# AIBluefisher/DReg-NeRF

Hardware: AMD Instinct MI355X
Metric: nerf_pairs_per_sec_regtr_fwd_bwd_128 (higher is better)
Workload: dtype bf16; 1 GPU; RegTR fwd+bwd+AdamW, shell-R synthetic pairs, 128^3 grids, 4 pairs (8 grids) per GPU per step, random-init weights; global_batch_pairs=4, resolution=128, fpn_head=active-set (identical results; rows around occupied voxels), parallelism=dp1

## Files before the change

dreg_nerf_amd/csrc/attention.hip:

```cpp
#include "common.h"

template <typename T> struct Frag;
template <> struct Frag<bf16_t> { bf16x8_t v; };
template <> struct Frag<float> { float v[8]; };

__device__ __forceinline__ f32x4_t mma(const Frag<bf16_t>& a, const Frag<bf16_t>& b, f32x4_t c) {
    return __builtin_amdgcn_mfma_f32_16x16x32_bf16(a.v, b.v, c, 0, 0, 0);
}
__device__ __forceinline__ f32x4_t mma(const Frag<float>& a, const Frag<float>& b, f32x4_t c) {
#pragma unroll
    for (int e = 0; e < 8; ++e) c = __builtin_amdgcn_mfma_f32_16x16x4f32(a.v[e], b.v[e], c, 0, 0, 0);
    return c;
}
__device__ __forceinline__ Frag<bf16_t> frag_row(const char* base, int rs, int row, int k0, bf16_t) {
    Frag<bf16_t> f; f.v = *reinterpret_cast<const bf16x8_t*>(base + row * rs + k0 * 2); return f;
}
__device__ __forceinline__ Frag<float> frag_row(const char* base, int rs, int row, int k0, float) {
    Frag<float> f;
    float4 lo = *reinterpret_cast<const float4*>(base + row * rs + k0 * 4);
    float4 hi = *reinterpret_cast<const float4*>(base + row * rs + k0 * 4 + 16);
    f.v[0] = lo.x; f.v[1] = lo.y; f.v[2] = lo.z; f.v[3] = lo.w; f.v[4] = hi.x; f.v[5] = hi.y; f.v[6] = hi.z; f.v[7] = hi.w;
    return f;
}
__device__ __forceinline__ Frag<bf16_t> frag_glob(const bf16_t* p, bool valid) {
    Frag<bf16_t> f;
    if (valid) f.v = *reinterpret_cast<const bf16x8_t*>(p); else f.v = (bf16x8_t){0, 0, 0, 0, 0, 0, 0, 0};
    return f;
}
__device__ __forceinline__ Frag<float> frag_glob(const float* p, bool valid) {
    Frag<float> f;
#pragma unroll
    for (int e = 0; e < 8; ++e) f.v[e] = valid ? p[e] : 0.f;
    return f;
}
struct AttnArgs {
    const void *q, *k, *v;
    void* o;
    float* lse;
    int Nq, Nk;
    int ldq, ldk, ldv, ldo;
    long hq, hk, hv, ho;
    float scale;
    const void* dout;
    float* dvec;
    void *dq, *dk, *dv;
    const int4* probs;
    int Rq;
};

struct Prob { int Nq, Nk; long q0, k0; };
__device__ __forceinline__ Prob get_prob(const AttnArgs& a) {
    Prob p; p.Nq = a.Nq; p.Nk = a.Nk; p.q0 = 0; p.k0 = 0;
    if (a.probs) { const int4 t = a.probs[blockIdx.z]; p.q0 = t.x; p.Nq = t.y; p.k0 = t.z; p.Nk = t.w; }
    return p;
}

template <typename T> __host__ __device__ constexpr int row_pad() { return sizeof(T) == 2 ? 32 : 16; }
template <typename T, int D>
struct TileRegs {
    static constexpr int GPR = D * sizeof(T) / 16, NL = (64 * GPR + 255) / 256;
    uint4 v[NL];
    __device__ __forceinline__ void fetch(const T* src, long ld, int row0, int nrows_valid, int tid) {
#pragma unroll
        for (int i = 0; i < NL; ++i) {
            const int q = tid + i * 256, r = q / GPR, g = q % GPR;
            v[i] = make_uint4(0, 0, 0, 0);
            if (q < 64 * GPR && row0 + r < nrows_valid) v[i] = *reinterpret_cast<const uint4*>(reinterpret_cast<const char*>(src + (long)(row0 + r) * ld) + g * 16);
        }
    }
    __device__ __forceinline__ void store(char* dst, int rs, int tid) const {
#pragma unroll
        for (int i = 0; i < NL; ++i) {
            const int q = tid + i * 256, r = q / GPR, g = q % GPR;
            if (q < 64 * GPR) *reinterpret_cast<uint4*>(dst + r * rs + g * 16) = v[i];
        }
    }
};
__device__ __forceinline__ Frag<bf16_t> frag_regs(const float (&v)[8], bf16_t) {
    typedef __attribute__((ext_vector_type(4))) uint32_t u32x4_t;
    const u32x4_t w = {f2bf2(v[0], v[1]), f2bf2(v[2], v[3]), f2bf2(v[4], v[5]), f2bf2(v[6], v[7])};
    Frag<bf16_t> f; f.v = __builtin_bit_cast(bf16x8_t, w); return f;
}
__device__ __forceinline__ Frag<float> frag_regs(const float (&v)[8], float) {
    Frag<float> f;
#pragma unroll
    for (int e = 0; e < 8; ++e) f.v[e] = v[e];
    return f;
}
__device__ __forceinline__ Frag<bf16_t> frag_colp(const char* base, int rs, int row_lo, int row_hi, int cb, int lane, bf16_t) {
    typedef __attribute__((address_space(3))) bf16x4_t* lds4_t;
    const int fi = lane & 15;
    const int off = (fi >> 2) * rs + (cb + (fi & 3) * 4) * 2;
    bf16x4_t lo = __builtin_amdgcn_ds_read_tr16_b64_v4i16((lds4_t)(base + row_lo * rs + off));
    bf16x4_t hi = __builtin_amdgcn_ds_read_tr16_b64_v4i16((lds4_t)(base + row_hi * rs + off));
    Frag<bf16_t> f; f.v = (bf16x8_t){lo[0], lo[1], lo[2], lo[3], hi[0], hi[1], hi[2], hi[3]};
    return f;
}
__device__ __forceinline__ Frag<float> frag_colp(const char* base, int rs, int row_lo, int row_hi, int cb, int lane, float) {
    const int fi = lane & 15;
    Frag<float> f;
#pragma unroll
    for (int e = 0; e < 8; ++e) f.v[e] = *reinterpret_cast<const float*>(base + (e < 4 ? row_lo + e : row_hi + e - 4) * rs + (cb + fi) * 4);
    return f;
}
__device__ __forceinline__ void store4(bf16_t* p, float a, float b, float c, float d) { *reinterpret_cast<uint2*>(p) = make_uint2(f2bf2(a, b), f2bf2(c, d)); }
__device__ __forceinline__ void store4(float* p, float a, float b, float c, float d) { *reinterpret_cast<float4*>(p) = make_float4(a, b, c, d); }
__device__ __forceinline__ float group4x_sum(float v) { v += __shfl_xor(v, 16, 64); v += __shfl_xor(v, 32, 64); return v; }
__device__ __forceinline__ float group4x_max(float v) { v = fmaxf(v, __shfl_xor(v, 16, 64)); return fmaxf(v, __shfl_xor(v, 32, 64)); }
constexpr float LOG2E = 1.4426950408889634f, LN2 = 0.6931471805599453f;

template <typename T, int D, bool XYZ>
__global__ __launch_bounds__(256) void attn_fwd_kernel(AttnArgs a)
{
    constexpr int DV = 32;
    constexpr int KRS = D * sizeof(T) + row_pad<T>(), VRS = XYZ ? 16 : DV * sizeof(T) + row_pad<T>();
    extern __shared__ __attribute__((aligned(16))) char smem[];
    constexpr int BUF = 64 * KRS + 64 * VRS;
    const int tid = threadIdx.x, lane = tid & 63, wave = tid >> 6;
    const int h = blockIdx.y;
    const Prob pb = get_prob(a);
    if (blockIdx.x * 64 >= pb.Nq) return;
    const int q0 = blockIdx.x * 64 + wave * 16;
    const T* Q = (const T*)a.q + h * a.hq + pb.q0 * a.ldq;
    const T* K = (const T*)a.k + h * a.hk + pb.k0 * a.ldk;
    const int fr = lane & 15, kg = lane >> 4;

    Frag<T> qf[D / 32];
#pragma unroll
    for (int kk = 0; kk < D / 32; ++kk) qf[kk] = frag_glob(Q + (long)(q0 + fr) * a.ldq + kk * 32 + kg * 8, q0 + fr < pb.Nq);
    const float c2 = a.scale * LOG2E;
    float m = -INFINITY, l = 0.f;
    f32x4_t o[2];
    float o3[3] = {0.f, 0.f, 0.f};
    o[0] = o[1] = (f32x4_t){0.f, 0.f, 0.f, 0.f};

    TileRegs<T, D> rk;
    TileRegs<T, DV> rv;
    float4 rx = make_float4(0, 0, 0, 0);
    const T* Vp = XYZ ? nullptr : (const T*)a.v + h * a.hv + pb.k0 * a.ldv;
    auto fetch = [&](int k0) {
        rk.fetch(K, a.ldk, k0, pb.Nk, tid);
        if constexpr (XYZ) {
            const float* x = (const float*)a.v + pb.k0 * 3;
            rx = make_float4(0, 0, 0, 0);
            if (tid < 64 && k0 + tid < pb.Nk) rx = make_float4(x[(long)(k0 + tid) * 3], x[(long)(k0 + tid) * 3 + 1], x[(long)(k0 + tid) * 3 + 2], 0.f);
        } else {
            rv.fetch(Vp, a.ldv, k0, pb.Nk, tid);
        }
    };
    auto stage = [&](int buf) {
        char* dK = smem + buf * BUF;
        rk.store(dK, KRS, tid);
        if constexpr (XYZ) { if (tid < 64) *reinterpret_cast<float4*>(dK + 64 * KRS + tid * 16) = rx; }
        else rv.store(dK + 64 * KRS, VRS, tid);
    };
    fetch(0);
    stage(0);
    if (64 < pb.Nk) fetch(64);
    for (int k0 = 0, buf = 0; k0 < pb.Nk; k0 += 64, buf ^= 1) {
        __syncthreads();
        if (k0 + 64 < pb.Nk) { stage(buf ^ 1); if (k0 + 128 < pb.Nk) fetch(k0 + 128); }
        const char* sK = smem + buf * BUF;
        const char* sV = sK + 64 * KRS;
        f32x4_t s[4];
#pragma unroll
        for (int t = 0; t < 4; ++t) {
            s[t] = (f32x4_t){0.f, 0.f, 0.f, 0.f};
#pragma unroll
            for (int kk = 0; kk < D / 32; ++kk) s[t] = mma(frag_row(sK, KRS, t * 16 + fr, kk * 32 + kg * 8, T()), qf[kk], s[t]);
        }
        if (k0 + 64 > pb.Nk) {
#pragma unroll
            for (int t = 0; t < 4; ++t)
#pragma unroll
                for (int r = 0; r < 4; ++r)
                    if (k0 + t * 16 + kg * 4 + r >= pb.Nk) s[t][r] = -INFINITY;
        }
        float mx = -INFINITY;
#pragma unroll
        for (int t = 0; t < 4; ++t)
#pragma unroll
            for (int r = 0; r < 4; ++r) mx = fmaxf(mx, s[t][r]);
        mx = group4x_max(mx) * c2;
        const float mn = fmaxf(m, mx);
        const float alpha = __builtin_amdgcn_exp2f(m - mn);
        float sum = 0.f;
#pragma unroll
        for (int t = 0; t < 4; ++t)
#pragma unroll
            for (int r = 0; r < 4; ++r) { s[t][r] = __builtin_amdgcn_exp2f(__builtin_fmaf(s[t][r], c2, -mn)); sum += s[t][r]; }
        l = l * alpha + sum;
        m = mn;
        if constexpr (XYZ) {
#pragma unroll
            for (int c = 0; c < 3; ++c) o3[c] *= alpha;
#pragma unroll
            for (int t = 0; t < 4; ++t)
#pragma unroll
                for (int r = 0; r < 4; ++r) {
                    const float4 x = *reinterpret_cast<const float4*>(sV + (t * 16 + kg * 4 + r) * 16);
                    o3[0] += s[t][r] * x.x; o3[1] += s[t][r] * x.y; o3[2] += s[t][r] * x.z;
                }
        } else {
#pragma unroll
            for (int r = 0; r < 4; ++r) { o[0][r] *= alpha; o[1][r] *= alpha; }
#pragma unroll
            for (int ks = 0; ks < 2; ++ks) {
                const float pv[8] = {s[2 * ks][0], s[2 * ks][1], s[2 * ks][2], s[2 * ks][3], s[2 * ks + 1][0], s[2 * ks + 1][1], s[2 * ks + 1][2], s[2 * ks + 1][3]};
                const Frag<T> pf = frag_regs(pv, T());
#pragma unroll
                for (int u = 0; u < 2; ++u) o[u] = mma(frag_colp(sV, VRS, ks * 32 + kg * 4, ks * 32 + 16 + kg * 4, u * 16, lane, T()), pf, o[u]);
            }
        }
    }
    l = group4x_sum(l);
    const float inv = 1.f / l;
    const int qr = q0 + fr;
    if constexpr (XYZ) {
        const float x = group4x_sum(o3[0]), y = group4x_sum(o3[1]), z = group4x_sum(o3[2]);
        if (kg == 0 && qr < pb.Nq) {
            float* op = (float*)a.o + ((long)h * a.Rq + pb.q0 + qr) * 3;
            op[0] = x * inv; op[1] = y * inv; op[2] = z * inv;
        }
    } else if (qr < pb.Nq) {
        T* op = (T*)a.o + h * a.ho + (pb.q0 + qr) * a.ldo + kg * 4;
#pragma unroll
        for (int u = 0; u < 2; ++u) store4(op + u * 16, o[u][0] * inv, o[u][1] * inv, o[u][2] * inv, o[u][3] * inv);
    }
    if (kg == 0 && qr < pb.Nq) a.lse[(long)h * a.Rq + pb.q0 + qr] = (m + __log2f(l)) * LN2;
}

template <typename T, int D, bool XYZ>
__global__ __launch_bounds__(256, (D > 32 ? 2 : 1)) void attn_bwd_dq_kernel(AttnArgs a)
{
    constexpr int DV = 32;
    constexpr int KRS = D * sizeof(T) + row_pad<T>(), VRS = XYZ ? 16 : DV * sizeof(T) + row_pad<T>();
    extern __shared__ __attribute__((aligned(16))) char smem[];
    constexpr int BUF = 64 * KRS + 64 * VRS;
    const int tid = threadIdx.x, lane = tid & 63, wave = tid >> 6;
    const int h = blockIdx.y;
    const Prob pb = get_prob(a);
    if (blockIdx.x * 64 >= pb.Nq) return;
    const int q0 = blockIdx.x * 64 + wave * 16;
    const T* Q = (const T*)a.q + h * a.hq + pb.q0 * a.ldq;
    const T* K = (const T*)a.k + h * a.hk + pb.k0 * a.ldk;
    const int fr = lane & 15, kg = lane >> 4;
    const int qr = q0 + fr;
    const bool qv = qr < pb.Nq;

    Frag<T> qf[D / 32];
#pragma unroll
    for (int kk = 0; kk < D / 32; ++kk) qf[kk] = frag_glob(Q + (long)qr * a.ldq + kk * 32 + kg * 8, qv);
    const float lse2 = qv ? a.lse[(long)h * a.Rq + pb.q0 + qr] * LOG2E : 0.f;
    float dvec, do3[3] = {0.f, 0.f, 0.f};
    Frag<T> dof;
    if constexpr (!XYZ) {
        const T* dO = (const T*)a.dout + h * a.ho + pb.q0 * a.ldo;
        const T* O = (const T*)a.o + h * a.ho + pb.q0 * a.ldo;
        dof = frag_glob(dO + (long)qr * a.ldo + kg * 8, qv);
        const Frag<T> of = frag_glob(O + (long)qr * a.ldo + kg * 8, qv);
        float part = 0.f;
        if constexpr (sizeof(T) == 2) {
#pragma unroll
            for (int e = 0; e < 8; ++e) part += bf2f((bf16_t)dof.v[e]) * bf2f((bf16_t)of.v[e]);
        } else {
#pragma unroll
            for (int e = 0; e < 8; ++e) part += dof.v[e] * of.v[e];
        }
        dvec = group4x_sum(part);
    } else {
        const float* dO = (const float*)a.dout + ((long)h * a.Rq + pb.q0 + qr) * 3;
        const float* O = (const float*)a.o + ((long)h * a.Rq + pb.q0 + qr) * 3;
        dvec = 0.f;
#pragma unroll
        for (int c = 0; c < 3; ++c) { do3[c] = qv ? dO[c] : 0.f; dvec += do3[c] * (qv ? O[c] : 0.f); }
    }
    if (kg == 0 && qv) a.dvec[(long)h * a.Rq + pb.q0 + qr] = dvec;
    const float c2 = a.scale * LOG2E;
    f32x4_t dq[D / 16];
#pragma unroll
    for (int u = 0; u < D / 16; ++u) dq[u] = (f32x4_t){0.f, 0.f, 0.f, 0.f};

    TileRegs<T, D> rk;
    TileRegs<T, DV> rv;
    float4 rx = make_float4(0, 0, 0, 0);
    const T* Vp = XYZ ? nullptr : (const T*)a.v + h * a.hv + pb.k0 * a.ldv;
    auto fetch = [&](int k0) {
        rk.fetch(K, a.ldk, k0, pb.Nk, tid);
        if constexpr (XYZ) {
            const float* x = (const float*)a.v + pb.k0 * 3;
            rx = make_float4(0, 0, 0, 0);
            if (tid < 64 && k0 + tid < pb.Nk) rx = make_float4(x[(long)(k0 + tid) * 3], x[(long)(k0 + tid) * 3 + 1], x[(long)(k0 + tid) * 3 + 2], 0.f);
        } else {
            rv.fetch(Vp, a.ldv, k0, pb.Nk, tid);
        }
    };
    auto stage = [&](int buf) {
        char* dK = smem + buf * BUF;
        rk.store(dK, KRS, tid);
        if constexpr (XYZ) { if (tid < 64) *reinterpret_cast<float4*>(dK + 64 * KRS + tid * 16) = rx; }
        else rv.store(dK + 64 * KRS, VRS, tid);
    };
    fetch(0);
    stage(0);
    if (64 < pb.Nk) fetch(64);
    for (int k0 = 0, buf = 0; k0 < pb.Nk; k0 += 64, buf ^= 1) {
        __syncthreads();
        if (k0 + 64 < pb.Nk) { stage(buf ^ 1); if (k0 + 128 < pb.Nk) fetch(k0 + 128); }
        const char* sK = smem + buf * BUF;
        const char* sV = sK + 64 * KRS;
#pragma unroll
        for (int ks = 0; ks < 2; ++ks) {
            float dsv[8];
#pragma unroll
            for (int tt = 0; tt < 2; ++tt) {
                const int t = 2 * ks + tt;
                f32x4_t s = (f32x4_t){0.f, 0.f, 0.f, 0.f};
#pragma unroll
                for (int kk = 0; kk < D / 32; ++kk) s = mma(frag_row(sK, KRS, t * 16 + fr, kk * 32 + kg * 8, T()), qf[kk], s);
                f32x4_t dp = (f32x4_t){0.f, 0.f, 0.f, 0.f};
                if constexpr (!XYZ) dp = mma(frag_row(sV, VRS, t * 16 + fr, kg * 8, T()), dof, dp);
                if (k0 + 64 > pb.Nk) {
#pragma unroll
                    for (int r = 0; r < 4; ++r)
                        if (k0 + t * 16 + kg * 4 + r >= pb.Nk) s[r] = -INFINITY;
                }
#pragma unroll
                for (int r = 0; r < 4; ++r) {
                    const int kr = t * 16 + kg * 4 + r;
                    const float p = __builtin_amdgcn_exp2f(__builtin_fmaf(s[r], c2, -lse2));
                    float dpv = dp[r];
                    if constexpr (XYZ) {
                        const float4 x = *reinterpret_cast<const float4*>(sV + kr * 16);
                        dpv = do3[0] * x.x + do3[1] * x.y + do3[2] * x.z;
                    }
                    dsv[tt * 4 + r] = p * (dpv - dvec);
                }
            }
            const Frag<T> df = frag_regs(dsv, T());
#pragma unroll
            for (int u = 0; u < D / 16; ++u) {
                dq[u] = mma(frag_colp(sK, KRS, ks * 32 + kg * 4, ks * 32 + 16 + kg * 4, u * 16, lane, T()), df, dq[u]);
                if (D > 32 && (u & 3) == 3) __builtin_amdgcn_sched_barrier(0);
            }
        }
    }
    if (qv) {
        T* dQ = (T*)a.dq + h * a.hq + (pb.q0 + qr) * a.ldq + kg * 4;
#pragma unroll
        for (int u = 0; u < D / 16; ++u) store4(dQ + u * 16, dq[u][0] * a.scale, dq[u][1] * a.scale, dq[u][2] * a.scale, dq[u][3] * a.scale);
    }
}

template <typename T, int D, bool XYZ>
__global__ __launch_bounds__(256, (D > 32 ? 2 : 1)) void attn_bwd_dkv_kernel(AttnArgs a)
{
    constexpr int DV = 32;
    constexpr int QRS = D * sizeof(T) + row_pad<T>(), ORS = XYZ ? 16 : DV * sizeof(T) + row_pad<T>();
    extern __shared__ __attribute__((aligned(16))) char smem[];
    constexpr int BUF = 64 * QRS + 64 * ORS + 128 * (int)sizeof(float);
    const int tid = threadIdx.x, lane = tid & 63, wave = tid >> 6;
    const int h = blockIdx.y;
    const Prob pb = get_prob(a);
    if (blockIdx.x * 64 >= pb.Nk) return;
    const int key0 = blockIdx.x * 64 + wave * 16;
    const T* Q = (const T*)a.q + h * a.hq + pb.q0 * a.ldq;
    const T* K = (const T*)a.k + h * a.hk + pb.k0 * a.ldk;
    const int fr = lane & 15, kg = lane >> 4;
    const int kr = key0 + fr;
    const bool kv = kr < pb.Nk;

    Frag<T> kf[D / 32], vf;
#pragma unroll
    for (int kk = 0; kk < D / 32; ++kk) kf[kk] = frag_glob(K + (long)kr * a.ldk + kk * 32 + kg * 8, kv);
    float x3[3] = {0.f, 0.f, 0.f};
    if constexpr (!XYZ) {
        vf = frag_glob((const T*)a.v + h * a.hv + (pb.k0 + (long)kr) * a.ldv + kg * 8, kv);
    } else {
#pragma unroll
        for (int c = 0; c < 3; ++c) x3[c] = kv ? ((const float*)a.v)[(pb.k0 + kr) * 3 + c] : 0.f;
    }
    const float c2 = a.scale * LOG2E;
    f32x4_t dk[D / 16], dvv[2];
#pragma unroll
    for (int u = 0; u < D / 16; ++u) dk[u] = (f32x4_t){0.f, 0.f, 0.f, 0.f};
    dvv[0] = dvv[1] = (f32x4_t){0.f, 0.f, 0.f, 0.f};

    TileRegs<T, D> rq;
    TileRegs<T, DV> ro;
    float4 rg = make_float4(0, 0, 0, 0);
    float rl = 0.f, rd = 0.f;
    const T* dOp = XYZ ? nullptr : (const T*)a.dout + h * a.ho + pb.q0 * a.ldo;
    auto fetch = [&](int q0) {
        rq.fetch(Q, a.ldq, q0, pb.Nq, tid);
        if constexpr (XYZ) {
            rg = make_float4(0, 0, 0, 0);
            if (tid < 64 && q0 + tid < pb.Nq) {
                const float* g = (const float*)a.dout + ((long)h * a.Rq + pb.q0 + q0 + tid) * 3;
                rg = make_float4(g[0], g[1], g[2], 0.f);
            }
        } else {
            ro.fetch(dOp, a.ldo, q0, pb.Nq, tid);
        }
        rl = rd = 0.f;
        if (tid < 64 && q0 + tid < pb.Nq) { rl = a.lse[(long)h * a.Rq + pb.q0 + q0 + tid] * LOG2E; rd = a.dvec[(long)h * a.Rq + pb.q0 + q0 + tid]; }
    };
    auto stage = [&](int buf) {
        char* dQ = smem + buf * BUF;
        rq.store(dQ, QRS, tid);
        if constexpr (XYZ) { if (tid < 64) *reinterpret_cast<float4*>(dQ + 64 * QRS + tid * 16) = rg; }
        else ro.store(dQ + 64 * QRS, ORS, tid);
        float* dL = reinterpret_cast<float*>(dQ + 64 * QRS + 64 * ORS);
        if (tid < 64) { dL[tid] = rl; dL[64 + tid] = rd; }
    };
    fetch(0);
    stage(0);
    if (64 < pb.Nq) fetch(64);
    for (int q0 = 0, buf = 0; q0 < pb.Nq; q0 += 64, buf ^= 1) {
        __syncthreads();
        if (q0 + 64 < pb.Nq) { stage(buf ^ 1); if (q0 + 128 < pb.Nq) fetch(q0 + 128); }
        const char* sQ = smem + buf * BUF;
        const char* sO = sQ + 64 * QRS;
        const float* sL = reinterpret_cast<const float*>(sO + 64 * ORS);
#pragma unroll
        for (int ks = 0; ks < 2; ++ks) {
            float pv[8], dsv[8];
#pragma unroll
            for (int tt = 0; tt < 2; ++tt) {
                const int t = 2 * ks + tt;
                f32x4_t s = (f32x4_t){0.f, 0.f, 0.f, 0.f};
#pragma unroll
                for (int kk = 0; kk < D / 32; ++kk) s = mma(frag_row(sQ, QRS, t * 16 + fr, kk * 32 + kg * 8, T()), kf[kk], s);
                f32x4_t dp = (f32x4_t){0.f, 0.f, 0.f, 0.f};
                if constexpr (!XYZ) dp = mma(frag_row(sO, ORS, t * 16 + fr, kg * 8, T()), vf, dp);
                const float4 l4 = *reinterpret_cast<const float4*>(sL + t * 16 + kg * 4);
                const float4 d4 = *reinterpret_cast<const float4*>(sL + 64 + t * 16 + kg * 4);
                const float lq[4] = {l4.x, l4.y, l4.z, l4.w}, dq_[4] = {d4.x, d4.y, d4.z, d4.w};
#pragma unroll
                for (int r = 0; r < 4; ++r) {
                    const int ql = t * 16 + kg * 4 + r;
                    const float p = __builtin_amdgcn_exp2f(__builtin_fmaf(s[r], c2, -lq[r]));
                    float dpv = dp[r];
                    if constexpr (XYZ) {
                        const float4 g = *reinterpret_cast<const float4*>(sO + ql * 16);
                        dpv = x3[0] * g.x + x3[1] * g.y + x3[2] * g.z;
                    }
                    pv[tt * 4 + r] = p;
                    dsv[tt * 4 + r] = p * (dpv - dq_[r]);
                }
            }
            const Frag<T> sf = frag_regs(dsv, T());
#pragma unroll
            for (int u = 0; u < D / 16; ++u) {
                dk[u] = mma(frag_colp(sQ, QRS, ks * 32 + kg * 4, ks * 32 + 16 + kg * 4, u * 16, lane, T()), sf, dk[u]);
                if (D > 32 && (u & 3) == 3) __builtin_amdgcn_sched_barrier(0);
            }
            if constexpr (!XYZ) {
                const Frag<T> pf = frag_regs(pv, T());
#pragma unroll
                for (int u = 0; u < 2; ++u) dvv[u] = mma(frag_colp(sO, ORS, ks * 32 + kg * 4, ks * 32 + 16 + kg * 4, u * 16, lane, T()), pf, dvv[u]);
            }
        }
    }
    if (kv) {
        T* dK = (T*)a.dk + h * a.hk + (pb.k0 + (long)kr) * a.ldk + kg * 4;
#pragma unroll
        for (int u = 0; u < D / 16; ++u) store4(dK + u * 16, dk[u][0] * a.scale, dk[u][1] * a.scale, dk[u][2] * a.scale, dk[u][3] * a.scale);
        if constexpr (!XYZ) {
            T* dV = (T*)a.dv + h * a.hv + (pb.k0 + (long)kr) * a.ldv + kg * 4;
            store4(dV, dvv[0][0], dvv[0][1], dvv[0][2], dvv[0][3]);
            store4(dV + 16, dvv[1][0], dvv[1][1], dvv[1][2], dvv[1][3]);
        }
    }
}

template <typename T, int D, bool XYZ>
static int launch_attn(const AttnArgs& a, int H, int mode, hipStream_t st, int nprob = 1, int maxq = 0, int maxk = 0)
{
    const int gq = ((a.probs ? maxq : a.Nq) + 63) / 64, gk = ((a.probs ? maxk : a.Nk) + 63) / 64;
    constexpr int DV = 32;
    const size_t krs = D * sizeof(T) + row_pad<T>(), vrs = XYZ ? 16 : DV * sizeof(T) + row_pad<T>();
    if (mode == 0) {
        const size_t lds = 2 * (64 * krs + 64 * vrs);
        if (lds > 65536) (void)hipFuncSetAttribute((const void*)attn_fwd_kernel<T, D, XYZ>, hipFuncAttributeMaxDynamicSharedMemorySize, (int)lds);
        hipLaunchKernelGGL((attn_fwd_kernel<T, D, XYZ>), dim3(gq, H, nprob), dim3(256), lds, st, a);
    } else if (mode == 1) {
        const size_t lds = 2 * (64 * krs + 64 * vrs);
        if (lds > 65536) (void)hipFuncSetAttribute((const void*)attn_bwd_dq_kernel<T, D, XYZ>, hipFuncAttributeMaxDynamicSharedMemorySize, (int)lds);
        hipLaunchKernelGGL((attn_bwd_dq_kernel<T, D, XYZ>), dim3(gq, H, nprob), dim3(256), lds, st, a);
    } else {
        const size_t lds = 2 * (64 * krs + 64 * vrs + 128 * sizeof(float));
        if (lds > 65536) (void)hipFuncSetAttribute((const void*)attn_bwd_dkv_kernel<T, D, XYZ>, hipFuncAttributeMaxDynamicSharedMemorySize, (int)lds);
        hipLaunchKernelGGL((attn_bwd_dkv_kernel<T, D, XYZ>), dim3(gk, H, nprob), dim3(256), lds, st, a);
    }
    DREG_LAUNCH_CHECK();
    return DREG_OK;
}

static int dispatch_attn(const AttnArgs& a, int H, int D, int xyz, int dtype, int mode, hipStream_t st, int nprob = 1, int maxq = 0, int maxk = 0)
{
    if (!a.probs && (a.Nq <= 0 || a.Nk <= 0)) return DREG_EINVAL;
    if (a.probs && (nprob <= 0 || maxq <= 0 || maxk <= 0)) return DREG_EINVAL;
    if (D == 32 && !xyz) return dtype == 0 ? launch_attn<bf16_t, 32, false>(a, H, mode, st, nprob, maxq, maxk) : launch_attn<float, 32, false>(a, H, mode, st, nprob, maxq, maxk);
    if (D == 256 && xyz) return dtype == 0 ? launch_attn<bf16_t, 256, true>(a, H, mode, st, nprob, maxq, maxk) : launch_attn<float, 256, true>(a, H, mode, st, nprob, maxq, maxk);
    return DREG_EINVAL;
}

extern "C" {

int dreg_mha_fwd(const void* q, const void* k, const void* v, void* o, float* lse, int Nq, int Nk, int H,
                 int ldq, int ldk, int ldv, int ldo, float scale, int dtype, void* stream)
{
    AttnArgs a = {};
    a.q = q; a.k = k; a.v = v; a.o = o; a.lse = lse; a.Nq = Nq; a.Nk = Nk;
    a.ldq = ldq; a.ldk = ldk; a.ldv = ldv; a.ldo = ldo; a.hq = a.hk = a.hv = a.ho = 32; a.scale = scale; a.Rq = Nq;
    return dispatch_attn(a, H, 32, 0, dtype, 0, (hipStream_t)stream);
}
int dreg_mha_bwd(const void* q, const void* k, const void* v, const void* o, const void* dout, const float* lse,
                 float* dvec, void* dq, void* dk, void* dv, int Nq, int Nk, int H,
                 int ldq, int ldk, int ldv, int ldo, float scale, int dtype, void* stream)
{
    AttnArgs a = {};
    a.q = q; a.k = k; a.v = v; a.o = (void*)o; a.lse = (float*)lse; a.Nq = Nq; a.Nk = Nk;
    a.ldq = ldq; a.ldk = ldk; a.ldv = ldv; a.ldo = ldo; a.hq = a.hk = a.hv = a.ho = 32; a.scale = scale;
    a.dout = dout; a.dvec = dvec; a.dq = dq; a.dk = dk; a.dv = dv; a.Rq = Nq;
    int rc = dispatch_attn(a, H, 32, 0, dtype, 1, (hipStream_t)stream);
    if (rc) return rc;
    return dispatch_attn(a, H, 32, 0, dtype, 2, (hipStream_t)stream);
}
int dreg_corr_attention_fwd(const void* q, const void* k, const float* xyz, float* out, float* lse, int L, int Nq, int Nk,
                            float scale, int dtype, void* stream)
{
    AttnArgs a = {};
    a.q = q; a.k = k; a.v = xyz; a.o = out; a.lse = lse; a.Nq = Nq; a.Nk = Nk;
    a.ldq = a.ldk = 256; a.hq = (long)Nq * 256; a.hk = (long)Nk * 256; a.scale = scale; a.Rq = Nq;
    return dispatch_attn(a, L, 256, 1, dtype, 0, (hipStream_t)stream);
}
int dreg_corr_attention_bwd(const void* q, const void* k, const float* xyz, const float* out, const float* dout,
                            const float* lse, float* dvec, void* dq, void* dk, int L, int Nq, int Nk,
                            float scale, int dtype, void* stream)
{
    AttnArgs a = {};
    a.q = q; a.k = k; a.v = xyz; a.o = (void*)out; a.lse = (float*)lse; a.Nq = Nq; a.Nk = Nk;
    a.ldq = a.ldk = 256; a.hq = (long)Nq * 256; a.hk = (long)Nk * 256; a.scale = scale;
    a.dout = dout; a.dvec = dvec; a.dq = dq; a.dk = dk; a.Rq = Nq;
    int rc = dispatch_attn(a, L, 256, 1, dtype, 1, (hipStream_t)stream);
    if (rc) return rc;
    return dispatch_attn(a, L, 256, 1, dtype, 2, (hipStream_t)stream);
}

int dreg_mha_varlen_fwd(const void* q, const void* k, const void* v, void* o, float* lse, const int* probs, int nprob,
                        int max_q, int max_k, int R, int H, int ldq, int ldk, int ldv, int ldo, float scale, int dtype, void* stream)
{
    AttnArgs a = {};
    a.q = q; a.k = k; a.v = v; a.o = o; a.lse = lse; a.probs = (const int4*)probs; a.Rq = R;
    a.ldq = ldq; a.ldk = ldk; a.ldv = ldv; a.ldo = ldo; a.hq = a.hk = a.hv = a.ho = 32; a.scale = scale;
    return dispatch_attn(a, H, 32, 0, dtype, 0, (hipStream_t)stream, nprob, max_q, max_k);
}
int dreg_mha_varlen_bwd(const void* q, const void* k, const void* v, const void* o, const void* dout, const float* lse,
                        float* dvec, void* dq, void* dk, void* dv, const int* probs, int nprob, int max_q, int max_k, int R, int H,
                        int ldq, int ldk, int ldv, int ldo, float scale, int dtype, void* stream)
{
    AttnArgs a = {};
    a.q = q; a.k = k; a.v = v; a.o = (void*)o; a.lse = (float*)lse; a.probs = (const int4*)probs; a.Rq = R;
    a.ldq = ldq; a.ldk = ldk; a.ldv = ldv; a.ldo = ldo; a.hq = a.hk = a.hv = a.ho = 32; a.scale = scale;
    a.dout = dout; a.dvec = dvec; a.dq = dq; a.dk = dk; a.dv = dv;
    int rc = dispatch_attn(a, H, 32, 0, dtype, 1, (hipStream_t)stream, nprob, max_q, max_k);
    if (rc) return rc;
    return dispatch_attn(a, H, 32, 0, dtype, 2, (hipStream_t)stream, nprob, max_q, max_k);
}
int dreg_corr_attention_varlen_fwd(const void* q, const void* k, const float* xyz, float* out, float* lse, const int* probs, int nprob,
                                   int max_q, int max_k, int L, int R, float scale, int dtype, void* stream)
{
    AttnArgs a = {};
    a.q = q; a.k = k; a.v = xyz; a.o = out; a.lse = lse; a.probs = (const int4*)probs; a.Rq = R;
    a.ldq = a.ldk = 256; a.hq = a.hk = (long)R * 256; a.scale = scale;
    return dispatch_attn(a, L, 256, 1, dtype, 0, (hipStream_t)stream, nprob, max_q, max_k);
}
int dreg_corr_attention_varlen_bwd(const void* q, const void* k, const float* xyz, const float* out, const float* dout,
                                   const float* lse, float* dvec, void* dq, void* dk, const int* probs, int nprob,
                                   int max_q, int max_k, int L, int R, float scale, int dtype, void* stream)
{
    AttnArgs a = {};
    a.q = q; a.k = k; a.v = xyz; a.o = (void*)out; a.lse = (float*)lse; a.probs = (const int4*)probs; a.Rq = R;
    a.ldq = a.ldk = 256; a.hq = a.hk = (long)R * 256; a.scale = scale;
    a.dout = dout; a.dvec = dvec; a.dq = dq; a.dk = dk;
    int rc = dispatch_attn(a, L, 256, 1, dtype, 1, (hipStream_t)stream, nprob, max_q, max_k);
    if (rc) return rc;
    return dispatch_attn(a, L, 256, 1, dtype, 2, (hipStream_t)stream, nprob, max_q, max_k);
}

}
```

dreg_nerf_amd/lib.py:

```python
import ctypes
import os
from ctypes import c_float, c_int, c_size_t, c_void_p

import torch

_HERE = os.path.dirname(os.path.abspath(__file__))
LIB_PATH = os.path.join(_HERE, "libdreg_nerf_hip.so")

DT_BF16 = 0
DT_F32 = 1

_lib = None


class DregError(RuntimeError):
    pass


def _sig(lib, name, restype, argtypes):
    fn = getattr(lib, name)
    fn.restype = restype
    fn.argtypes = argtypes
    return fn

# ... 119 lines not shown
    "dreg_exec_set_timing": (None, [P, I]),
    "dreg_exec_read_timings": (I, [P, P, P, I]),
    "dreg_exec_forward": (I, [P, P, Z, P, P, P, I, I, P]),
    "dreg_exec_backward": (I, [P, P, Z, P, P, P, P, I, P, P]),
    "dreg_exec_backward_range": (I, [P, P, Z, P, P, P, P, I, P, P, I, I, I]),
    "dreg_mha_fwd": (I, [P] * 5 + [I] * 7 + [F, I, P]),
    "dreg_mha_bwd": (I, [P] * 10 + [I] * 7 + [F, I, P]),
    "dreg_corr_attention_fwd": (I, [P] * 5 + [I] * 3 + [F, I, P]),
    "dreg_corr_attention_bwd": (I, [P] * 9 + [I] * 3 + [F, I, P]),
    "dreg_mha_varlen_fwd": (I, [P] * 6 + [I] * 9 + [F, I, P]),
    "dreg_mha_varlen_bwd": (I, [P] * 11 + [I] * 9 + [F, I, P]),
    "dreg_corr_attention_varlen_fwd": (I, [P] * 6 + [I] * 5 + [F, I, P]),
    "dreg_corr_attention_varlen_bwd": (I, [P] * 10 + [I] * 5 + [F, I, P]),
    "dreg_layernorm_fwd": (I, [P] * 6 + [I, I, F, I, P]),
    "dreg_layernorm_bwd_workspace_bytes": (Z, [I]),
    "dreg_layernorm_bwd": (I, [P] * 8 + [I] * 5 + [P]),
    "dreg_layernorm_bwd_add": (I, [P] * 9 + [I] * 4 + [P]),
    "dreg_layernorm_fwd2": (I, [P, P, P, P, I, P, P, P, I, I, F, P]),
    "dreg_layernorm_bwd_parts": (I, [P] * 10 + [I, I, I, P]),
    "dreg_layernorm_bwd_blocks": (I, [I]),
    "dreg_layernorm_bwd_final_batched": (I, [P, I, P]),
    "dreg_overlap_bwd_acc": (I, [P, P, P, P, P, P, P, P, I, P, I, P]),
    "dreg_colsum_rows_per_chunk": (I, [Z]),
    "dreg_colsum_batched": (I, [P, I, I, I, P]),
    "dreg_brick_supported": (I, [I] * 6),
    "dreg_conv3_brick_pack_bytes": (Z, [I, I]),
    "dreg_pack_conv_weight_brick": (I, [P, P, I, I, I, P]),
    "dreg_brick_tiles_workspace_bytes": (Z, [I] * 4),
    "dreg_brick_tiles_build": (I, [P, I, I, I, I, I, I, P, Z, P, P, P, P, P, P]),
    "dreg_conv3_brick": (I, [P, P, P, P, P, P, I, P, P, P] + [I] * 11 + [P]),
    "dreg_ps_num_params": (I, []),
    "dreg_ps_num_linears": (I, []),
    "dreg_ps_create": (P, [P]),
    "dreg_ps_destroy": (None, [P]),
    "dreg_ps_set_fuse": (None, [P, I]),
    "dreg_ps_set_timing": (None, [P, I]),
    "dreg_ps_read_timings": (I, [P, P, P, I]),
    "dreg_ps_arena_bytes": (Z, [P, I]),
    "dreg_ps_panel_fwd": (I, [P] * 13 + [I, I, I, I, F, P]),
    "dreg_ps_panel_bwd": (I, [P] * 12 + [I, I, I, P]),
    "dreg_ps_forward": (I, [P, P, Z, P, P, P, P, P, P, I, I, I, P, P, P, P]),
    "dreg_ps_backward": (I, [P, P, Z, P, P, P, P, P, P, I, I, I, P, P, P, P, P, P, P, P, P, I]),
    "dreg_posenc_sine": (I, [P, P, I, F, F, P]),
    "dreg_overlap_fwd": (I, [P, P, P, P, I, P]),
    "dreg_overlap_bwd_workspace_bytes": (Z, [I]),
    "dreg_overlap_bwd": (I, [P] * 8 + [I, P]),
    "dreg_relu_bwd": (I, [P, P, P, Z, I, I, I, P]),
    "dreg_weighted_kabsch": (I, [P, P, P, P, I, I, F, P]),
    "dreg_weighted_kabsch_pairs": (I, [P, P, P, P, P, I, I, I, F, P]),
    "dreg_weighted_kabsch_bwd": (I, [P] * 7 + [I, I, F, P]),
    "dreg_weighted_kabsch_pairs_bwd": (I, [P] * 7 + [I, I, I, F, P]),
    "dreg_reg_point_losses": (I, [P] * 10 + [I, I, I, I, F, F, F, P]),
    "dreg_infonce_nn": (I, [P] * 7 + [I, I, F, P]),
    "dreg_infonce_rows": (I, [P] * 10 + [I, I, F, F, I, P]),
    "dreg_reg_losses_final": (I, [P] * 6 + [I, I, F, F, F, F, F, P]),
    "dreg_nerf_cont_deferred": (I, [P] * 5 + [I, I, I, F, F, F, F, P]),
    "dreg_halfspace_labels": (I, [P, P, P, P, I, I, P]),
    "dreg_voxel_downsample_workspace_bytes": (Z, [I]),
    "dreg_voxel_downsample_fwd": (I, [P] * 11 + [Z, I, I, I, F, P]),
    "dreg_voxel_downsample_bwd": (I, [P, P, P, P, I, I, P]),
    "dreg_voxel_downsample_plan": (I, [P] * 11 + [Z, I, I, F, P]),
    "dreg_voxel_downsample_plan_frozen": (I, [P] * 11 + [Z, I, I, F, P, P]),
    "dreg_voxel_segment_mean": (I, [P] * 5 + [I, I, P]),
    "dreg_grad_norm": (I, [P, P, P, Z, P]),
    "dreg_adamw_step": (I, [P] * 5 + [Z] + [F] * 5 + [I, F, P]),
    "dreg_ngp_level_table": (ctypes.c_uint32, [F, I, I, P, P, P, P, P]),
    "dreg_f32_to_f16": (I, [P, P, Z, P]),
    "dreg_ngp_density_fwd": (I, [P] * 6 + [P] * 5 + [P, I, P]),
    "dreg_ngp_rgb_mean_fwd": (I, [P] * 6 + [I, I, P]),
    "dreg_ngp_dir_bias": (I, [P, P, P, I, P]),
    "dreg_ngp_alpha_keep": (I, [P, P, P, I, F, F, P]),
    "dreg_ngp_density_fwd_contract": (I, [P] * 6 + [P] * 5 + [P, I, I, P]),
    "dreg_ngp_density_fwd_ws": (I, [P] * 6 + [P] * 5 + [P, I, I, P, Z, P, I, P]),
    "dreg_grid_sample_points_ordered": (I, [P, P, P, P, P, I, I, I, P, I, P]),
    "dreg_grid_x_order_workspace_bytes": (Z, [I, I, I]),
    "dreg_grid_x_order": (I, [P, P, P, P, Z, I, I, I, I, P]),
    "dreg_grid_occupied_workspace_bytes": (Z, [I, I, I]),
    "dreg_grid_occupied_totals": (P, [P, I, I, I]),
    "dreg_grid_occupied_count": (I, [P, P, Z, I, I, I, P]),
    "dreg_grid_occupied_build": (I, [P, P, P, P, P, P, P, P, I, I, I, I, P]),
    "dreg_ngp_density_keep_fwd_ws": (I, [P] * 6 + [P] * 5 + [P, I, I, P, Z, P, I] + [P, P, F, F, P]),
    "dreg_grid_write_kept": (I, [P, P, P, P, P, P, P, P, I, I, I, I, P]),
    "dreg_ngp_density_workspace_bytes": (Z, [I]),
    "dreg_ngp_rgb_dir_fwd": (I, [P] * 6 + [I, P]),
    "dreg_grid_scatter7": (I, [P] * 6 + [I, P]),
    "dreg_grid_sample_points": (I, [P, P, P, I, I, I, P, I, P]),
    "dreg_surface_visibility": (I, [P] * 7 + [P] * 5 + [P, P, P] + [I] * 5 + [F, F, F, F, P]),
    "dreg_surface_visibility_queue": (I, [P] * 7 + [P] * 5 + [P, P, P] + [I] * 5 + [F, F, F, F, P, P, P]),
    "dreg_occupancy_coarse_bits": (I, [P, P, I, I, I, P]),
    "dreg_surface_visibility_desc_bytes": (Z, []),
    "dreg_surface_visibility_fill_desc": (I, [P] + [P] * 7 + [P] * 5 + [P, P, P] + [I] * 5 + [F, F, F, F, P, P]),
    "dreg_surface_visibility_multi": (I, [P, I, ctypes.c_long, P]),
    "dreg_surface_visibility_multi_waves": (I, [P, I, ctypes.c_long, I, P]),
    "dreg_ngp_render": (I, [P, P, ctypes.c_long, P, I, I, I, P] + [P] * 6 + [P] * 5 + [P, P, P] + [F] * 5 + [P] + [P] * 6),
    "dreg_ngp_render_pair": (I, [ctypes.c_long] + ([P, P, P, I, I, I, P] + [P] * 6 + [P] * 5 + [P, P, P] + [F] * 4 + [P]) * 2 + [F, F, P] + [P] * 7),
    "dreg_ngp_render_scene": (I, [ctypes.c_long, I, P, F, F, P] + [P] * 7),
    "dreg_ngp_render_train": (I, [P, P, P, ctypes.c_long, P, I, I, I, P] + [P] * 6 + [P] * 5 + [P, P, P] + [F] * 5 + [P] + [P] * 6),
    "dreg_ngp_render_bwd_workspace_bytes": (Z, [ctypes.c_long]),
    "dreg_ngp_render_bwd": (I, [P, P, P, ctypes.c_long, P, I, I, I, P, P, P] + [P] * 5 + [P, P, P] + [F] * 5 + [P, P, P, P, P, Z, P]),
    "dreg_ngp_adam_step": (I, [P] * 5 + [Z, F, F, F, F, I, P]),
    "dreg_image_metrics_workspace_bytes": (Z, [I, I, I, I]),
    "dreg_image_metrics": (I, [P, P, I, I, I, I, P] + [P] * 6 + [P, Z, P]),
    "dreg_ngp_density_grad": (I, [P] * 7 + [P] * 5 + [P, I, I, P]),
    "dreg_icp_workspace_bytes": (Z, [I, I]),
    "dreg_icp_refine": (I, [P, I, P, P, P, P, I, P, F, I, I, I, P, F, I] + [ctypes.c_double] * 3 + [P, P, P, P, P, Z, P]),
    "dreg_pose_ransac_workspace_bytes": (Z, [I, I]),
    "dreg_pose_ransac": (I, [P, P, I, P, I, F, F, P, Z, P, P, P, P, P, P, P]),
    "dreg_pose_inliers": (I, [P, P, I, P, F, P, P, P]),
    "dreg_mc_table": (I, [P, P]),
    "dreg_mc_workspace_bytes": (Z, [I, I, I]),
    "dreg_mc_count": (I, [P, I, I, I, F, P, Z, P, P]),
    "dreg_mc_emit": (I, [P, I, I, I, F, P, P, P, Z, P, P, I, I, P]),
    "dreg_pair_density": (I, [P, ctypes.c_long, P, P, I, I, I] + ([P, I, I, I] + [P] * 3 + [P] * 5 + [P] * 3) * 2 + [P, F] + [P] * 5 + [P]),
}


PROBE_SIGNATURES = {
    "dreg_conv1_bnrelu_a_probe": (I, [P, P, P, P, I, I, I, I, I, I, P]),
    "dreg_conv_set_glds": (None, [I]),
    "dreg_conv_set_wgrad_splits": (None, [I]),
    "dreg_conv_set_wgrad_big": (None, [I]),
    "dreg_conv_igemm_probe": (None, [I]),
    "dreg_conv_set_igemm_ap": (None, [I]),
    "dreg_conv_set_igemm_ap256": (None, [I]),
    "dreg_conv_set_pointwise_rmw_cin": (None, [I]),
    "dreg_conv_igemm_probe_read": (I, [P]),
    "dreg_conv_set_wgrad_pipe": (None, [I]),
    "dreg_conv_wgrad_probe_read": (I, [P]),
    "dreg_conv_set_wgrad_ring": (None, [I]),
    "dreg_conv_set_wgrad_rows_fast": (None, [I]),
    "dreg_conv_set_row_splits": (None, [I]),
    "dreg_conv_set_glds_stages": (None, [I]),
    "dreg_conv_set_wgrad_target_blocks": (None, [I]),
    "dreg_conv_set_narrow_small": (None, [I]),
    "dreg_bn_set_debug_skip": (None, [I]),
    "dreg_bn_set_store_g": (None, [I]),
    "dreg_bn_set_small_regs": (None, [I]),
    "dreg_sstem_set_pool_blocks": (None, [I]),
    "dreg_voxel_set_own_sort": (None, [I]),
    "dreg_conv_set_bn_stats_epilogue": (None, [I]),
    "dreg_conv3_halo_set_variant": (None, [I]),
    "dreg_conv3_halo64_set": (None, [I]),
    "dreg_conv3_halo_set_prof": (None, [P]),
    "dreg_bn_set_small_max_voxels": (None, [I]),
    "dreg_ngp_set_rgb_chunks": (None, [I]),
    "dreg_ngp_set_density_unroll": (None, [I]),
    "dreg_ngp_set_xcd_levels": (None, [I]),
    "dreg_visibility_set_waves": (None, [I]),
    "dreg_visibility_set_pass_bound": (I, [ctypes.c_long]),
    "dreg_render_set_waves": (None, [I]),
    "dreg_render_pair_set_waves": (None, [I]),
    "dreg_render_bwd_set_waves": (None, [I]),
    "dreg_render_scene_set_waves": (None, [I]),
}
PROBE_LIB_PATH = os.path.join(_HERE, "libdreg_nerf_hip_probe.so")
_probe_lib = None


class ExecOpts(ctypes.Structure):
    _fields_ = [(n, c_int) for n in ("sparse_grads", "bn_batch_tails", "fuse_stem", "sparse_stem", "fold_res_bn", "fold_splitk", "group_wgrad",
                                     "s2_accumulate", "fuse_bn_stats", "brick", "defer_head_pg", "persistent_deep", "guard", "pointwise_stream")] + [("reserved", c_int * 2)]


SCENE_MAX_BLOCKS = 4


class SceneBlock(ctypes.Structure):
    _fields_ = ([("origins", P), ("viewdirs", P), ("binary", P), ("rx", c_int), ("ry", c_int), ("rz", c_int), ("coarse_bits", P)] +
                [(n, P) for n in ("table", "w1", "w2", "cw1", "cw2", "cw3", "offset", "size", "res", "scale", "hashed", "roi_aabb", "scene_aabb", "model_aabb")] +
                [(n, c_float) for n in ("near_plane", "far_plane", "render_step_size", "alpha_thre")] + [("center", P)])


def load_probe():
    global _probe_lib
    if _probe_lib is None:
        if not os.path.exists(PROBE_LIB_PATH):
            raise DregError(f"{PROBE_LIB_PATH} not found: build it with `python -m dreg_nerf_amd.build`")
        lib = ctypes.CDLL(PROBE_LIB_PATH)
        for name, (rt, at) in list(SIGNATURES.items()) + list(PROBE_SIGNATURES.items()):
            _sig(lib, name, rt, at)
        _probe_lib = lib
    return _probe_lib


def use_probe():
    global _lib
    _lib = load_probe()
    return _lib


class probe:

    def __init__(self):
        self._restore = []

    def __enter__(self):
        global _lib
        self._saved = _lib
        _lib = load_probe()
        self.lib = _lib
        return self

    def set(self, name, value, default):
        getattr(self.lib, name)(value)
        self._restore.append((name, default))

    def __getattr__(self, name):
        return getattr(self.__dict__["lib"], name)

    def __exit__(self, *exc):
        global _lib
        for name, default in reversed(self._restore):
            getattr(self.lib, name)(default)
        _lib = self._saved
        return False


def load():
    global _lib
    if _lib is None:
        if not os.path.exists(LIB_PATH):
            raise DregError(
                f"{LIB_PATH} not found: build it with `python -m dreg_nerf_amd.build` "
                "(hipcc --offload-arch=gfx950); dreg_nerf_amd has no CPU/eager fallback")
        lib = ctypes.CDLL(LIB_PATH)
        for name, (rt, at) in SIGNATURES.items():
            _sig(lib, name, rt, at)
        _lib = lib
    return _lib


def declared_symbols():
    return list(SIGNATURES.keys())


def probe_symbols():
    return list(PROBE_SIGNATURES.keys())


def ptr(t):
    if t is None:
        return None
    assert t.is_contiguous(), "non-contiguous tensor handed to the C ABI"
    return t.data_ptr()


def _floats(n, v):
    return (c_float * n)(*[float(t) for t in (v.reshape(-1).tolist() if torch.is_tensor(v) else v)])


def f6(v):
    return _floats(6, v)


def f3(v):
    return _floats(3, v)


_raw_stream = getattr(torch._C, "_cuda_getCurrentRawStream", None)


def stream():
    if _raw_stream is not None:
        return _raw_stream(torch.cuda.current_device())
    return torch.cuda.current_stream().cuda_stream


_DEBUG_SYNC = bool(int(os.environ.get("DREG_DEBUG_SYNC", "0")))


def check(rc, name):
    if rc != 0:
        raise DregError(f"{name} failed with code {rc}")
    if _DEBUG_SYNC:
        import sys
        print(f"[dreg] {name} launched", file=sys.stderr, flush=True)
        torch.cuda.synchronize()


def dt_of(t: torch.Tensor) -> int:
    if t.dtype == torch.bfloat16:
        return DT_BF16
    if t.dtype == torch.float32:
        return DT_F32
    raise DregError(f"unsupported dtype {t.dtype}")


def torch_dtype(dt: int):
    return torch.bfloat16 if dt == DT_BF16 else torch.float32


def to_device_async(data, dtype, device):
    t = torch.tensor(data, dtype=dtype)
    if device.type != "cuda":
        return t
    return t.pin_memory().to(device, non_blocking=True)
```

include/dreg_nerf_probe.h:

```cpp
#ifndef DREG_NERF_PROBE_H
#define DREG_NERF_PROBE_H
#ifdef __cplusplus
extern "C" {
#endif

void dreg_conv3_halo_set_variant(int variant);
void dreg_conv3_halo64_set(int v);
void dreg_conv3_halo_set_prof(void* u64_buf_64x8x5);
void dreg_conv_set_glds(int enable);
int dreg_conv1_bnrelu_a_probe(const void* in, const void* wt_packed, void* out, const float* a_scale_shift, int B, int D, int H, int W, int Cin, int Cout, void* stream);
void dreg_conv_set_wgrad_splits(int splits);
void dreg_conv_set_wgrad_rows_fast(int enable);
void dreg_conv_set_row_splits(int on);
void dreg_conv_set_wgrad_ring(int mode);
int dreg_conv_wgrad_probe_read(unsigned long long* out8);
void dreg_conv_set_wgrad_pipe(int enable);
void dreg_conv_set_igemm_ap(int max_tiles);
void dreg_conv_set_pointwise_rmw_cin(int max_cin);
void dreg_conv_set_igemm_ap256(int on);
void dreg_conv_igemm_probe(int enable);
int dreg_conv_igemm_probe_read(unsigned long long* out6);
void dreg_conv_set_wgrad_big(int mode);
void dreg_conv_set_glds_stages(int stages);
void dreg_conv_set_wgrad_target_blocks(int blocks);
void dreg_bn_set_small_max_voxels(int v);
void dreg_sstem_set_pool_blocks(int n);
void dreg_voxel_set_own_sort(int on);
void dreg_conv_set_bn_stats_epilogue(int on);
void dreg_bn_set_store_g(int enable);
void dreg_bn_set_small_regs(int enable);
void dreg_bn_set_debug_skip(int mask);
void dreg_ngp_set_rgb_chunks(int on);
void dreg_ngp_set_density_unroll(int n);
void dreg_ngp_set_xcd_levels(int on);
int dreg_visibility_set_pass_bound(long passes);
void dreg_visibility_set_waves(int n);
void dreg_render_set_waves(int n);
void dreg_render_pair_set_waves(int n);
void dreg_render_scene_set_waves(int n);
void dreg_render_bwd_set_waves(int n);
void dreg_conv_set_narrow_small(int on);

#ifdef __cplusplus
}
#endif
#endif
```

Measured before the change: 263.4 pairs/s.

## Merge attention backward dQ and dK/dV into one launch with in-kernel delta

Attention backward is now one kernel whose grid covers both key blocks (dK/dV role) and query blocks (dQ role), replacing two sequential launches. The dK/dV role computes the rowwise dot(dO, O) term itself, using DPP quad swaps to reduce it, instead of reading a precomputed dvec. This removes one launch and the serialization between the two passes, and lets both roles fill the GPU together. In exchange the dK/dV role does redundant delta work, and the merged kernel uses different occupancy bounds. A probe knob restores the split path.

Result: no change. 263.3 pairs/s (median of 2 runs) (-0.0%).

```diff
diff --git a/dreg_nerf_amd/csrc/attention.hip b/dreg_nerf_amd/csrc/attention.hip
--- a/dreg_nerf_amd/csrc/attention.hip
+++ b/dreg_nerf_amd/csrc/attention.hip
@@ -107,6 +107,9 @@
 __device__ __forceinline__ void store4(float* p, float a, float b, float c, float d) { *reinterpret_cast<float4*>(p) = make_float4(a, b, c, d); }
 __device__ __forceinline__ float group4x_sum(float v) { v += __shfl_xor(v, 16, 64); v += __shfl_xor(v, 32, 64); return v; }
 __device__ __forceinline__ float group4x_max(float v) { v = fmaxf(v, __shfl_xor(v, 16, 64)); return fmaxf(v, __shfl_xor(v, 32, 64)); }
+template <int PERM> __device__ __forceinline__ float quad_swap(float v) {
+    return __builtin_bit_cast(float, __builtin_amdgcn_mov_dpp(__builtin_bit_cast(int, v), PERM, 0xF, 0xF, true));
+}
 constexpr float LOG2E = 1.4426950408889634f, LN2 = 0.6931471805599453f;
 
 template <typename T, int D, bool XYZ>
@@ -231,7 +234,7 @@
 }
 
 template <typename T, int D, bool XYZ>
-__global__ __launch_bounds__(256, (D > 32 ? 2 : 1)) void attn_bwd_dq_kernel(AttnArgs a)
+__device__ __forceinline__ void attn_bwd_dq_role(const AttnArgs& a, const int bx)
 {
     constexpr int DV = 32;
     constexpr int KRS = D * sizeof(T) + row_pad<T>(), VRS = XYZ ? 16 : DV * sizeof(T) + row_pad<T>();
@@ -240,8 +243,8 @@
     const int tid = threadIdx.x, lane = tid & 63, wave = tid >> 6;
     const int h = blockIdx.y;
     const Prob pb = get_prob(a);
-    if (blockIdx.x * 64 >= pb.Nq) return;
-    const int q0 = blockIdx.x * 64 + wave * 16;
+    if (bx * 64 >= pb.Nq) return;
+    const int q0 = bx * 64 + wave * 16;
     const T* Q = (const T*)a.q + h * a.hq + pb.q0 * a.ldq;
     const T* K = (const T*)a.k + h * a.hk + pb.k0 * a.ldk;
     const int fr = lane & 15, kg = lane >> 4;
@@ -352,8 +355,8 @@
     }
 }
 
-template <typename T, int D, bool XYZ>
-__global__ __launch_bounds__(256, (D > 32 ? 2 : 1)) void attn_bwd_dkv_kernel(AttnArgs a)
+template <typename T, int D, bool XYZ, bool OWN_DVEC>
+__device__ __forceinline__ void attn_bwd_dkv_role(const AttnArgs& a, const int bx)
 {
     constexpr int DV = 32;
     constexpr int QRS = D * sizeof(T) + row_pad<T>(), ORS = XYZ ? 16 : DV * sizeof(T) + row_pad<T>();
@@ -362,8 +365,8 @@
     const int tid = threadIdx.x, lane = tid & 63, wave = tid >> 6;
     const int h = blockIdx.y;
     const Prob pb = get_prob(a);
-    if (blockIdx.x * 64 >= pb.Nk) return;
-    const int key0 = blockIdx.x * 64 + wave * 16;
+    if (bx * 64 >= pb.Nk) return;
+    const int key0 = bx * 64 + wave * 16;
     const T* Q = (const T*)a.q + h * a.hq + pb.q0 * a.ldq;
     const T* K = (const T*)a.k + h * a.hk + pb.k0 * a.ldk;
     const int fr = lane & 15, kg = lane >> 4;
@@ -390,20 +393,36 @@
     TileRegs<T, DV> ro;
     float4 rg = make_float4(0, 0, 0, 0);
     float rl = 0.f, rd = 0.f;
+    Frag<T> fd, fo;
+    float o3[3] = {0.f, 0.f, 0.f};
     const T* dOp = XYZ ? nullptr : (const T*)a.dout + h * a.ho + pb.q0 * a.ldo;
+    const T* Op = XYZ ? nullptr : (const T*)a.o + h * a.ho + pb.q0 * a.ldo;
     auto fetch = [&](int q0) {
         rq.fetch(Q, a.ldq, q0, pb.Nq, tid);
         if constexpr (XYZ) {
             rg = make_float4(0, 0, 0, 0);
+            if constexpr (OWN_DVEC) o3[0] = o3[1] = o3[2] = 0.f;
             if (tid < 64 && q0 + tid < pb.Nq) {
                 const float* g = (const float*)a.dout + ((long)h * a.Rq + pb.q0 + q0 + tid) * 3;
                 rg = make_float4(g[0], g[1], g[2], 0.f);
+                if constexpr (OWN_DVEC) {
+                    const float* o = (const float*)a.o + ((long)h * a.Rq + pb.q0 + q0 + tid) * 3;
+                    o3[0] = o[0]; o3[1] = o[1]; o3[2] = o[2];
+                }
             }
         } else {
             ro.fetch(dOp, a.ldo, q0, pb.Nq, tid);
+            if constexpr (OWN_DVEC) {
+                const int r = q0 + (tid >> 2);
+                fo = frag_glob(Op + (long)r * a.ldo + (tid & 3) * 8, r < pb.Nq);
+                if constexpr (sizeof(T) != 2) fd = frag_glob(dOp + (long)r * a.ldo + (tid & 3) * 8, r < pb.Nq);
+            }
         }
         rl = rd = 0.f;
-        if (tid < 64 && q0 + tid < pb.Nq) { rl = a.lse[(long)h * a.Rq + pb.q0 + q0 + tid] * LOG2E; rd = a.dvec[(long)h * a.Rq + pb.q0 + q0 + tid]; }
+        if (tid < 64 && q0 + tid < pb.Nq) {
+            rl = a.lse[(long)h * a.Rq + pb.q0 + q0 + tid] * LOG2E;
+            if constexpr (!OWN_DVEC) rd = a.dvec[(long)h * a.Rq + pb.q0 + q0 + tid];
+        }
     };
     auto stage = [&](int buf) {
         char* dQ = smem + buf * BUF;
@@ -411,7 +430,29 @@
         if constexpr (XYZ) { if (tid < 64) *reinterpret_cast<float4*>(dQ + 64 * QRS + tid * 16) = rg; }
         else ro.store(dQ + 64 * QRS, ORS, tid);
         float* dL = reinterpret_cast<float*>(dQ + 64 * QRS + 64 * ORS);
-        if (tid < 64) { dL[tid] = rl; dL[64 + tid] = rd; }
+        if constexpr (!OWN_DVEC) {
+            if (tid < 64) { dL[tid] = rl; dL[64 + tid] = rd; }
+        } else if constexpr (XYZ) {
+            rd = 0.f;
+            rd += rg.x * o3[0]; rd += rg.y * o3[1]; rd += rg.z * o3[2];
+            if (tid < 64) { dL[tid] = rl; dL[64 + tid] = rd; }
+        } else {
+            float part = 0.f;
+            if constexpr (sizeof(T) == 2) {
+                typedef __attribute__((ext_vector_type(4))) uint32_t u32x4_t;
+                const u32x4_t w = {ro.v[0].x, ro.v[0].y, ro.v[0].z, ro.v[0].w};
+                fd.v = __builtin_bit_cast(bf16x8_t, w);
+#pragma unroll
+                for (int e = 0; e < 8; ++e) part += bf2f((bf16_t)fd.v[e]) * bf2f((bf16_t)fo.v[e]);
+            } else {
+#pragma unroll
+                for (int e = 0; e < 8; ++e) part += fd.v[e] * fo.v[e];
+            }
+            part += quad_swap<0xB1>(part);
+            part += quad_swap<0x4E>(part);
+            if ((tid & 3) == 0) dL[64 + (tid >> 2)] = part;
+            if (tid < 64) dL[tid] = rl;
+        }
     };
     fetch(0);
     stage(0);
@@ -474,6 +515,20 @@
     }
 }
 
+template <typename T, int D> constexpr int attn_bwd_waves() { return D > 32 ? (sizeof(T) == 2 ? 2 : 1) : (sizeof(T) == 2 ? 5 : 1); }
+template <typename T, int D, bool XYZ>
+__global__ __launch_bounds__(256, (attn_bwd_waves<T, D>())) void attn_bwd_kernel(AttnArgs a, int gk)
+{
+    if ((int)blockIdx.x < gk) attn_bwd_dkv_role<T, D, XYZ, true>(a, blockIdx.x);
+    else attn_bwd_dq_role<T, D, XYZ>(a, blockIdx.x - gk);
+}
+template <typename T, int D, bool XYZ>
+__global__ __launch_bounds__(256, (D > 32 ? 2 : 1)) void attn_bwd_dq_kernel(AttnArgs a) { attn_bwd_dq_role<T, D, XYZ>(a, blockIdx.x); }
+template <typename T, int D, bool XYZ>
+__global__ __launch_bounds__(256, (D > 32 ? 2 : 1)) void attn_bwd_dkv_kernel(AttnArgs a) { attn_bwd_dkv_role<T, D, XYZ, false>(a, blockIdx.x); }
+
+DREG_KNOB(int, g_attn_bwd_split, 0);
+
 template <typename T, int D, bool XYZ>
 static int launch_attn(const AttnArgs& a, int H, int mode, hipStream_t st, int nprob = 1, int maxq = 0, int maxk = 0)
 {
@@ -488,10 +543,14 @@
         const size_t lds = 2 * (64 * krs + 64 * vrs);
         if (lds > 65536) (void)hipFuncSetAttribute((const void*)attn_bwd_dq_kernel<T, D, XYZ>, hipFuncAttributeMaxDynamicSharedMemorySize, (int)lds);
         hipLaunchKernelGGL((attn_bwd_dq_kernel<T, D, XYZ>), dim3(gq, H, nprob), dim3(256), lds, st, a);
-    } else {
+    } else if (mode == 2) {
         const size_t lds = 2 * (64 * krs + 64 * vrs + 128 * sizeof(float));
         if (lds > 65536) (void)hipFuncSetAttribute((const void*)attn_bwd_dkv_kernel<T, D, XYZ>, hipFuncAttributeMaxDynamicSharedMemorySize, (int)lds);
         hipLaunchKernelGGL((attn_bwd_dkv_kernel<T, D, XYZ>), dim3(gk, H, nprob), dim3(256), lds, st, a);
+    } else {
+        const size_t lds = 2 * (64 * krs + 64 * vrs + 128 * sizeof(float));
+        if (lds > 65536) (void)hipFuncSetAttribute((const void*)attn_bwd_kernel<T, D, XYZ>, hipFuncAttributeMaxDynamicSharedMemorySize, (int)lds);
+        hipLaunchKernelGGL((attn_bwd_kernel<T, D, XYZ>), dim3(gk + gq, H, nprob), dim3(256), lds, st, a, gk);
     }
     DREG_LAUNCH_CHECK();
     return DREG_OK;
@@ -505,8 +564,19 @@
     if (D == 256 && xyz) return dtype == 0 ? launch_attn<bf16_t, 256, true>(a, H, mode, st, nprob, maxq, maxk) : launch_attn<float, 256, true>(a, H, mode, st, nprob, maxq, maxk);
     return DREG_EINVAL;
 }
+static int dispatch_attn_bwd(const AttnArgs& a, int H, int D, int xyz, int dtype, hipStream_t st, int nprob = 1, int maxq = 0, int maxk = 0)
+{
+    if (!g_attn_bwd_split) return dispatch_attn(a, H, D, xyz, dtype, 3, st, nprob, maxq, maxk);
+    int rc = dispatch_attn(a, H, D, xyz, dtype, 1, st, nprob, maxq, maxk);
+    if (rc) return rc;
+    return dispatch_attn(a, H, D, xyz, dtype, 2, st, nprob, maxq, maxk);
+}
 
 extern "C" {
+
+#ifdef DREG_PROBE
+void dreg_attn_set_bwd_split(int split) { g_attn_bwd_split = split ? 1 : 0; }
+#endif
 
 int dreg_mha_fwd(const void* q, const void* k, const void* v, void* o, float* lse, int Nq, int Nk, int H,
                  int ldq, int ldk, int ldv, int ldo, float scale, int dtype, void* stream)
@@ -524,9 +594,7 @@
     a.q = q; a.k = k; a.v = v; a.o = (void*)o; a.lse = (float*)lse; a.Nq = Nq; a.Nk = Nk;
     a.ldq = ldq; a.ldk = ldk; a.ldv = ldv; a.ldo = ldo; a.hq = a.hk = a.hv = a.ho = 32; a.scale = scale;
     a.dout = dout; a.dvec = dvec; a.dq = dq; a.dk = dk; a.dv = dv; a.Rq = Nq;
-    int rc = dispatch_attn(a, H, 32, 0, dtype, 1, (hipStream_t)stream);
-    if (rc) return rc;
-    return dispatch_attn(a, H, 32, 0, dtype, 2, (hipStream_t)stream);
+    return dispatch_attn_bwd(a, H, 32, 0, dtype, (hipStream_t)stream);
 }
 int dreg_corr_attention_fwd(const void* q, const void* k, const float* xyz, float* out, float* lse, int L, int Nq, int Nk,
                             float scale, int dtype, void* stream)
@@ -544,9 +612,7 @@
     a.q = q; a.k = k; a.v = xyz; a.o = (void*)out; a.lse = (float*)lse; a.Nq = Nq; a.Nk = Nk;
     a.ldq = a.ldk = 256; a.hq = (long)Nq * 256; a.hk = (long)Nk * 256; a.scale = scale;
     a.dout = dout; a.dvec = dvec; a.dq = dq; a.dk = dk; a.Rq = Nq;
-    int rc = dispatch_attn(a, L, 256, 1, dtype, 1, (hipStream_t)stream);
-    if (rc) return rc;
-    return dispatch_attn(a, L, 256, 1, dtype, 2, (hipStream_t)stream);
+    return dispatch_attn_bwd(a, L, 256, 1, dtype, (hipStream_t)stream);
 }
 
 int dreg_mha_varlen_fwd(const void* q, const void* k, const void* v, void* o, float* lse, const int* probs, int nprob,
@@ -565,9 +631,7 @@
     a.q = q; a.k = k; a.v = v; a.o = (void*)o; a.lse = (float*)lse; a.probs = (const int4*)probs; a.Rq = R;
     a.ldq = ldq; a.ldk = ldk; a.ldv = ldv; a.ldo = ldo; a.hq = a.hk = a.hv = a.ho = 32; a.scale = scale;
     a.dout = dout; a.dvec = dvec; a.dq = dq; a.dk = dk; a.dv = dv;
-    int rc = dispatch_attn(a, H, 32, 0, dtype, 1, (hipStream_t)stream, nprob, max_q, max_k);
-    if (rc) return rc;
-    return dispatch_attn(a, H, 32, 0, dtype, 2, (hipStream_t)stream, nprob, max_q, max_k);
+    return dispatch_attn_bwd(a, H, 32, 0, dtype, (hipStream_t)stream, nprob, max_q, max_k);
 }
 int dreg_corr_attention_varlen_fwd(const void* q, const void* k, const float* xyz, float* out, float* lse, const int* probs, int nprob,
                                    int max_q, int max_k, int L, int R, float scale, int dtype, void* stream)
@@ -585,9 +649,7 @@
     a.q = q; a.k = k; a.v = xyz; a.o = (void*)out; a.lse = (float*)lse; a.probs = (const int4*)probs; a.Rq = R;
     a.ldq = a.ldk = 256; a.hq = a.hk = (long)R * 256; a.scale = scale;
     a.dout = dout; a.dvec = dvec; a.dq = dq; a.dk = dk;
-    int rc = dispatch_attn(a, L, 256, 1, dtype, 1, (hipStream_t)stream, nprob, max_q, max_k);
-    if (rc) return rc;
-    return dispatch_attn(a, L, 256, 1, dtype, 2, (hipStream_t)stream, nprob, max_q, max_k);
-}
-
-}
+    return dispatch_attn_bwd(a, L, 256, 1, dtype, (hipStream_t)stream, nprob, max_q, max_k);
+}
+
+}
diff --git a/dreg_nerf_amd/lib.py b/dreg_nerf_amd/lib.py
--- a/dreg_nerf_amd/lib.py
+++ b/dreg_nerf_amd/lib.py
@@ -295,6 +295,7 @@
     "dreg_render_pair_set_waves": (None, [I]),
     "dreg_render_bwd_set_waves": (None, [I]),
     "dreg_render_scene_set_waves": (None, [I]),
+    "dreg_attn_set_bwd_split": (None, [I]),
 }
 PROBE_LIB_PATH = os.path.join(_HERE, "libdreg_nerf_hip_probe.so")
 _probe_lib = None
diff --git a/include/dreg_nerf_probe.h b/include/dreg_nerf_probe.h
--- a/include/dreg_nerf_probe.h
+++ b/include/dreg_nerf_probe.h
@@ -40,6 +40,7 @@
 void dreg_render_scene_set_waves(int n);
 void dreg_render_bwd_set_waves(int n);
 void dreg_conv_set_narrow_small(int on);
+void dreg_attn_set_bwd_split(int split);
 
 #ifdef __cplusplus
 }
```
